# MomentsInGraphics/vulkan_renderer

Hardware: NVIDIA H100
Metric: Msamples/s (pixels x spp) at 1920x1080x64spp; achieved HBM GB/s vs roofline (higher is better)
Workload: dtype f32

## Files before the change

__graft_entry__.py:

```python
import hashlib
import os
import shutil
import subprocess
import sys

ROOT = os.path.dirname(os.path.abspath(__file__))
PKG = os.path.join(ROOT, "vulkan_renderer_b200")
CSRC = os.path.join(PKG, "csrc")
LIB = os.path.join(PKG, "libvkr_b200.so")
NVCC = shutil.which("nvcc") or "/usr/local/cuda/bin/nvcc"
HOST_CXX = "/usr/bin/g++"

NVCC_FLAGS = [
	"-gencode", "arch=compute_90a,code=sm_90a", "-lineinfo", "-O3", "-std=c++17",
	"-fmad=false", "-prec-div=true", "-prec-sqrt=true", "-ftz=false",
	"-ccbin", HOST_CXX, "-Xcompiler", "-fPIC,-O2,-ffp-contract=off,-fopenmp,-Wall,-Wno-unused-function",
	"-I", os.path.join(ROOT, "include"),
]
NVCC_FLAGS += [f for f in os.environ.get("VKR_EXTRA_NVCC", "").split() if f]
CUDA_INCLUDE =os.path.join(os.path.dirname(os.path.dirname(os.path.realpath(NVCC))), "include")
HOST_FLAGS = ["-O2", "-std=c++17", "-fPIC", "-ffp-contract=off", "-fopenmp", "-Wall", "-Wno-unused-function", "-Wno-unused-result",
	"-I", os.path.join(ROOT, "include"), "-I", os.path.join(ROOT, "shim"), "-I", CUDA_INCLUDE]
CUDA_SOURCES = ["vkr_gbuffer_kernel.cu", "vkr_api.cu", "vkr_exchange.cu", "vkr_lbvh_gpu.cu"]
SHADING_KERNEL_BOUNDS = [4, 5, 6, 7, 8]
RELATED_WORK_KERNEL_BOUNDS = [3, 4, 5, 6, 7]
HOST_SOURCES = ["vkr_host.cpp", "vkr_bvh.cpp", "vkr_lbvh.cpp", "vkr_output.cpp", "vkr_textures.cpp"]


def _run(cmd, **kw):
	proc = subprocess.run(cmd, stdout=subprocess.PIPE, stderr=subprocess.STDOUT, text=True, **kw)
	if proc.returncode != 0:
		sys.stderr.write(proc.stdout)
		raise RuntimeError("command failed: %s" % " ".join(cmd))
	return proc.stdout


def _newer(target, sources):
	if not os.path.exists(target):
		return True
	t = os.path.getmtime(target)
	return any(os.path.getmtime(s) > t for s in sources)


def _all_headers():
	out = []
	for d in (CSRC, os.path.join(ROOT, "include"), os.path.join(ROOT, "shim"), os.path.join(ROOT, "shim", "vulkan")):
		if os.path.isdir(d):
			out += [os.path.join(d, f) for f in os.listdir(d) if f.endswith((".h", ".cuh", ".inc"))]
	return out


def build_library(verbose=False):
	obj_dir = os.path.join(PKG, "build")
	os.makedirs(obj_dir, exist_ok=True)
	headers = _all_headers()
	objects = []
	sources = [(s, [], s + ".o") for s in CUDA_SOURCES + HOST_SOURCES if os.path.exists(os.path.join(CSRC, s))]
	sources += [("vkr_shading_kernel.cu", ["-DVKR_MAXP_TU=%d" % k], "vkr_shading_kernel_maxp%d.cu.o" % k) for k in SHADING_KERNEL_BOUNDS]
	sources += [("vkr_shading_kernel.cu", ["-DVKR_MAXP_TU=5", "-DVKR_TRACE_STATS=1"], "vkr_shading_kernel_stats_maxp5.cu.o")]
	sources += [("vkr_textured_light_kernel.cu", ["-DVKR_MAXP_TU=%d" % k], "vkr_textured_light_kernel_maxp%d.cu.o" % k) for k in SHADING_KERNEL_BOUNDS]
	sources += [("vkr_related_work_kernel.cu", ["-DVKR_MAXV_TU=%d" % k], "vkr_related_work_kernel_maxv%d.cu.o" % k) for k in RELATED_WORK_KERNEL_BOUNDS]
	sources += [("vkr_textured_related_work_kernel.cu", ["-DVKR_MAXV_TU=%d" % k], "vkr_textured_related_work_kernel_maxv%d.cu.o" % k) for k in RELATED_WORK_KERNEL_BOUNDS]
	procs = []
	for src, defines, obj_name in sources:
		path = os.path.join(CSRC, src)
		obj = os.path.join(obj_dir, obj_name)
		objects.append(obj)
		if _newer(obj, [path] + headers):
			if src.endswith(".cu"):
				cmd = [NVCC] + NVCC_FLAGS + defines + (["-Xptxas", "-v"] if verbose else []) + ["-c", path, "-o", obj]
			else:
				cmd = [HOST_CXX] + HOST_FLAGS + ["-c", path, "-o", obj]
			procs.append((obj_name, subprocess.Popen(cmd, stdout=subprocess.PIPE, stderr=subprocess.STDOUT, text=True)))
	failed = False
	for src, proc in procs:
		out, _ = proc.communicate()
		if proc.returncode != 0:
			sys.stderr.write("---- %s\n%s\n" % (src, out))
			failed = True
		elif verbose:
			sys.stdout.write("---- %s\n%s\n" % (src, out))
	if failed:
		raise RuntimeError("nvcc failed")
	if _newer(LIB, objects):
		_run([NVCC, "-shared", "-o", LIB] + objects + ["-ccbin", HOST_CXX, "-Xcompiler", "-fopenmp", "-lgomp", "-cudart", "static"])
	return LIB


def build_device_on_host():
	src = os.path.join(ROOT, "tests", "device_on_host.cpp")
	out = os.path.join(ROOT, "tests", "build", "libdevice_on_host.so")
	os.makedirs(os.path.dirname(out), exist_ok=True)
	if _newer(out, [src] + _all_headers()):
		_run([HOST_CXX, "-O2", "-std=c++17", "-fPIC", "-shared", "-ffp-contract=off", "-mfma", "-mavx2", "-mf16c", "-Wall", "-Wno-unused-function", "-Wno-unknown-pragmas",
			"-I", CSRC, src, "-o", out])
	return out


def build_oracle():
	_run(["make", "-C", os.path.join(ROOT, "oracle")])
	ref_recipe = os.path.join(ROOT, "oracle", "build_ref.py")
	if os.path.isdir("/root/reference/src") and os.path.exists(ref_recipe):
		_run([sys.executable, ref_recipe])


def build():
	build_library()
	build_oracle()
	build_device_on_host()
	sys.path.insert(0, ROOT)
	import vulkan_renderer_b200


def smoke():
	sys.path.insert(0, ROOT)
	from tests import harness as H
	from vulkan_renderer_b200 import api
	if not os.path.exists(LIB):
		raise RuntimeError("libvkr_b200.so has not been built; there is no CPU fallback")
	width, height = 128, 96
	info = H.dataset("cornell")
	oi = H.OracleInputs(info)
	frame = H.open_frame(info, cuda_device=0)
	try:
		frame.configure(sample_count=2, strategy=api.STRATEGY_DIFFUSE_SPECULAR_MIS, heuristic=api.MIS_OPTIMAL_CLAMPED, trace_shadow_rays=1)
		constants = frame.constants(width, height)
		vis, gb = frame.gbuffer_host(width, height)
		out = frame.shade_host(width, height, gb)
		ref, rays = oi.shade(H.oracle_config(frame, width, height), constants, gb)
	finally:
		frame.close()
	cmp = H.compare_radiance(out, ref, rel=1.0e-5)
	print("smoke: %dx%d Cornell frame, %d oracle shadow rays, %s" % (width, height, rays, cmp))
	if cmp["bad_pixels"] or cmp["nan_mismatch"] or not np_any_lit(out):
		raise RuntimeError("smoke test failed: %s" % cmp)


def np_any_lit(image):
	import numpy as np
	return bool(np.isfinite(image).all() and (image[..., :3] > 0).any())


if __name__ == "__main__":
	build_library(verbose="-v" in sys.argv)
	build_oracle()
	build_device_on_host()
	print("built", LIB)
```

vulkan_renderer_b200/csrc/vkr_ray_stream.cuh:

```cuda
#pragma once
#include "vkr_trace.cuh"
#include "vkr_anchor.cuh"

namespace vkr {

#ifndef VKR_ANCHORED
#define VKR_ANCHORED 0
#endif

#ifndef VKR_RING
#define VKR_RING 256
#endif
constexpr int kRing = VKR_RING;
constexpr unsigned kFullMask = 0xffffffffu;
#ifndef VKR_TRACE_GROUPS
#define VKR_TRACE_GROUPS 2
#endif
constexpr int kShadeWarps = 4, kTraceWarps = 4 * VKR_TRACE_GROUPS;
constexpr unsigned kPending = 0xffu;
#ifndef VKR_BVH_WIDTH
#define VKR_BVH_WIDTH 2
#endif
#ifndef VKR_NODE_LOOP_MIN_LANES
#define VKR_NODE_LOOP_MIN_LANES 16
#endif
constexpr int kNodeLoopMinLanes = VKR_NODE_LOOP_MIN_LANES;
#ifndef VKR_REFILL_MIN_LANES
#define VKR_REFILL_MIN_LANES 1
#endif
#ifndef VKR_LEAN_NODE_STEP
#define VKR_LEAN_NODE_STEP (!VKR_ANCHORED && VKR_BVH_WIDTH == 2)
#endif
#ifndef VKR_LEAF_ONCE
#define VKR_LEAF_ONCE 0
#endif
#ifndef VKR_LEAF_POSTPONE
#define VKR_LEAF_POSTPONE 1
#endif
#ifndef VKR_STACK_TOP_IN_REGISTER
#define VKR_STACK_TOP_IN_REGISTER 0
#endif
#ifndef VKR_TRACE_RELOAD_RAY
#define VKR_TRACE_RELOAD_RAY 0
#endif
#ifndef VKR_SHADING_LOCKSTEP
#define VKR_SHADING_LOCKSTEP 0
#endif
#ifndef VKR_NODE_LOOP_CHECK_EVERY
#define VKR_NODE_LOOP_CHECK_EVERY 1
#endif
VKR_DEV void shading_lockstep_barrier() {
#if defined(__CUDA_ARCH__)
	asm volatile("bar.sync 1, 128;" ::: "memory");
#endif
}
#ifndef VKR_QUANTISED_NODES
#define VKR_QUANTISED_NODES 0
#endif
#ifndef VKR_INTERLEAVED_NODES
#define VKR_INTERLEAVED_NODES (!VKR_ANCHORED && !VKR_QUANTISED_NODES && VKR_BVH_WIDTH == 2)
#endif
#if VKR_ANCHORED && VKR_BVH_WIDTH != 2
#error "anchored rays walk node pairs"
#endif
#if VKR_LEAN_NODE_STEP && (VKR_ANCHORED || VKR_BVH_WIDTH != 2 || VKR_STACK_TOP_IN_REGISTER)
#error "the predicated node step: not with anchored rays, 4-wide nodes or the stack top in a register (-DVKR_LEAN_NODE_STEP=0)"
#endif
#if VKR_INTERLEAVED_NODES && (VKR_ANCHORED || VKR_QUANTISED_NODES || VKR_BVH_WIDTH != 2)
#error "interleaved node pairs: not with anchored rays, quantised pairs or 4-wide nodes"
#endif
#ifndef VKR_RESOLVE_SLEEP_NS
#define VKR_RESOLVE_SLEEP_NS 512
#endif

#ifdef VKR_TRACE_STATS
#define VKR_STAT(x) (++(x))
#define VKR_STAT_ADD(x, n) ((x) += (n))
#else
#define VKR_STAT(x) ((void) 0)
#define VKR_STAT_ADD(x, n) ((void) 0)
#endif
VKR_DEV void stat_flush(unsigned long long* stats, int index, unsigned value) {
#if defined(VKR_TRACE_STATS) && defined(__CUDA_ARCH__)
	value = __reduce_add_sync(kFullMask, value);
	if ((threadIdx.x & 31) == 0 && value != 0u && stats) atomicAdd(stats + index, (unsigned long long) value);
#endif
}

enum : int {
	S_DX = 0, S_DY = kRing, S_DZ = 2 * kRing, S_TMAX = 3 * kRing,
	S_CX = 4 * kRing, S_CY = 5 * kRing, S_CZ = 6 * kRing,
	S_OX = 7 * kRing, S_OY = 8 * kRing, S_OZ = 9 * kRing
};
VKR_DEV constexpr int stream_bytes_at(bool optimal) { return (optimal ? 10 : 7) * kRing; }
VKR_DEV constexpr int stream_origin_at(bool optimal) { return stream_bytes_at(optimal) + 2 * kRing / 4; }
VKR_DEV constexpr int stream_control_at(bool optimal) { return stream_origin_at(optimal) + 96; }
VKR_DEV constexpr int stream_mask_at(bool optimal) { return stream_control_at(optimal) + 4; }
VKR_DEV constexpr int stream_path_at(bool optimal) { return stream_mask_at(optimal) + kRing; }
VKR_DEV constexpr int stream_cone_at(bool optimal) { return stream_path_at(optimal) + 32 * (kPathLevels + 2); }
VKR_DEV constexpr size_t stream_floats_per_warp(bool optimal) { return VKR_ANCHORED ? (size_t) stream_cone_at(optimal) + 6 * 32 : (size_t) stream_control_at(optimal) + 4; }

VKR_DEV uint32_t smem_addr(const void* p) { return (uint32_t) __cvta_generic_to_shared(p); }
VKR_DEV uint32_t lds_u32(uint32_t a) { uint32_t v; asm volatile("ld.shared.u32 %0, [%1];" : "=r"(v) : "r"(a) : "memory"); return v; }
VKR_DEV void sts_u32(uint32_t a, uint32_t v) { asm volatile("st.shared.u32 [%0], %1;" :: "r"(a), "r"(v) : "memory"); }
VKR_DEV float lds_f(uint32_t a) { float v; asm volatile("ld.shared.f32 %0, [%1];" : "=f"(v) : "r"(a) : "memory"); return v; }
VKR_DEV void sts_f(uint32_t a, float v) { asm volatile("st.shared.f32 [%0], %1;" :: "r"(a), "f"(v) : "memory"); }
VKR_DEV unsigned lds_u8(uint32_t a) { unsigned v; asm volatile("ld.shared.u8 %0, [%1];" : "=r"(v) : "r"(a) : "memory"); return v; }
VKR_DEV void sts_u8(uint32_t a, unsigned v) { asm volatile("st.shared.u8 [%0], %1;" :: "r"(a), "r"(v) : "memory"); }
VKR_DEV int ld_acquire(uint32_t a) { int v; asm volatile("ld.acquire.cta.shared::cta.b32 %0, [%1];" : "=r"(v) : "r"(a) : "memory"); return v; }
VKR_DEV void st_release(uint32_t a, int v) { asm volatile("st.release.cta.shared::cta.b32 [%0], %1;" :: "r"(a), "r"(v) : "memory"); }
VKR_DEV unsigned ld_acquire_u8(uint32_t a) { unsigned v; asm volatile("ld.acquire.cta.shared::cta.u8 %0, [%1];" : "=r"(v) : "r"(a) : "memory"); return v; }
VKR_DEV void st_release_u8(uint32_t a, unsigned v) { asm volatile("st.release.cta.shared::cta.u8 [%0], %1;" :: "r"(a), "r"(v) : "memory"); }
VKR_DEV int atom_add_shared(uint32_t a, int v) { int old; asm volatile("atom.relaxed.cta.shared::cta.add.s32 %0, [%1], %2;" : "=r"(old) : "r"(a), "r"(v) : "memory"); return old; }

struct ray_producer {
	uint32_t base;
	int fill;
	int resolved;
#ifdef VKR_TRACE_STATS
	unsigned stat_resolve_polls, stat_candidates;
#endif
	bool cone_set;
	bool lockstep;
};

struct pixel_sum {
	f3 color;
	f3 light;
	float inv_samples;
	unsigned submit_parity, resolve_parity;
	bool pushed;
};
VKR_DEV void close_light(pixel_sum& acc) {
	acc.color = acc.color + acc.light * acc.inv_samples;
	acc.light = make3(0.0f, 0.0f, 0.0f);
}

template <bool OPTIMAL>
VKR_DEV void resolve_chunk(ray_producer& q, int lane, pixel_sum& acc) {
	const uint32_t bytes = q.base + 4u * stream_bytes_at(OPTIMAL);
	const int first = q.resolved;
	const int n = min(32, q.fill - first);
	const uint32_t slot = (uint32_t) (first + lane) & (kRing - 1);
	const bool valid = lane < n;
	while (true) {
		const unsigned r = valid ? ld_acquire_u8(bytes + kRing + slot) : 0u;
		if (!__any_sync(kFullMask, r == kPending)) break;
		VKR_STAT(q.stat_resolve_polls);
		__nanosleep(VKR_RESOLVE_SLEEP_NS);
	}
	const unsigned own = valid ? (lds_u8(bytes + slot) & 31u) : 32u;
	unsigned mine = __ballot_sync(kFullMask, valid);
#pragma unroll
	for (int b = 0; b != 5; ++b) {
		const unsigned bits = __ballot_sync(kFullMask, (own >> b) & 1u);
		mine &= ((lane >> b) & 1) ? bits : ~bits;
	}
	while (mine) {
		const uint32_t e = (uint32_t) (first + __ffs(mine) - 1) & (kRing - 1);
		mine &= mine - 1;
		const uint32_t a = q.base + 4u * e;
		const unsigned parity = lds_u8(bytes + e) & 32u;
		if (parity != acc.resolve_parity) { close_light(acc); acc.resolve_parity = parity; }
		if (!lds_u8(bytes + kRing + e)) acc.light = acc.light + make3(lds_f(a + 4u * S_CX), lds_f(a + 4u * S_CY), lds_f(a + 4u * S_CZ));
		else if (OPTIMAL) acc.light = acc.light + make3(lds_f(a + 4u * S_OX), lds_f(a + 4u * S_OY), lds_f(a + 4u * S_OZ));
	}
	q.resolved = first + n;
	__syncwarp(kFullMask);
}

#define OPTIMAL_STREAM_HAS_CONE(q) ((q).cone_set)
template <bool TRACE, bool OPTIMAL>
VKR_DEV void set_light_cone(ray_producer& q, int lane, bool on, f3 origin, const unsigned char* vertices, int vertex_count, const float4* __restrict__ nodes) {
#if VKR_ANCHORED
	if constexpr (TRACE) {
		q.cone_set = false;
		if (on) {
			const light_cone c = make_light_cone(origin, vertices, vertex_count);
			if (c.enabled) {
				const uint32_t path = q.base + 4u * (uint32_t) stream_path_at(OPTIMAL) + 4u * (uint32_t) lane;
				const int count = (int) lds_u32(path + 128u * (uint32_t) (kPathLevels + 1));
				const uint32_t siblings = cull_siblings(nodes, origin, c, count, [&](int k) { return lds_u32(path + 128u * (uint32_t) k); });
				const uint32_t ca = q.base + 4u * (uint32_t) stream_cone_at(OPTIMAL) + 4u * (uint32_t) lane;
				sts_f(ca, c.axis.x); sts_f(ca + 128u, c.axis.y); sts_f(ca + 256u, c.axis.z); sts_f(ca + 384u, c.cos2_valid); sts_f(ca + 512u, c.len2_valid); sts_u32(ca + 640u, siblings);
				q.cone_set = true;
			}
		}
	}
#endif
}
template <bool TRACE, bool OPTIMAL>
VKR_DEV void submit(ray_producer& q, int lane, bool has, bool need_trace, f3 dir_world, float tmax, f3 c_visible, f3 c_occluded, pixel_sum& acc, bool finish) {
	if constexpr (!TRACE) {
		if (has) {
			if (need_trace) acc.light = acc.light + c_visible;
			else if (OPTIMAL) acc.light = acc.light + c_occluded;
		}
		if (finish) close_light(acc);
	}
	else {
		const bool push = has && (need_trace || OPTIMAL);
		if (has) VKR_STAT(q.stat_candidates);
		const unsigned mask = __ballot_sync(kFullMask, push);
		if (mask) {
			const int k = __popc(mask);
			while (q.fill + k - q.resolved > kRing) resolve_chunk<OPTIMAL>(q, lane, acc);
			if (push) {
				const uint32_t e = (uint32_t) (q.fill + __popc(mask & ((1u << lane) - 1u))) & (kRing - 1);
				const uint32_t a = q.base + 4u * e;
				sts_f(a + 4u * S_DX, dir_world.x); sts_f(a + 4u * S_DY, dir_world.y); sts_f(a + 4u * S_DZ, dir_world.z); sts_f(a + 4u * S_TMAX, tmax);
				sts_f(a + 4u * S_CX, c_visible.x); sts_f(a + 4u * S_CY, c_visible.y); sts_f(a + 4u * S_CZ, c_visible.z);
				if (OPTIMAL) { sts_f(a + 4u * S_OX, c_occluded.x); sts_f(a + 4u * S_OY, c_occluded.y); sts_f(a + 4u * S_OZ, c_occluded.z); }
				const uint32_t bytes = q.base + 4u * stream_bytes_at(OPTIMAL);
				sts_u8(bytes + e, (unsigned) lane | acc.submit_parity | (need_trace ? 0u : 128u));
				sts_u8(bytes + kRing + e, kPending);
#if VKR_ANCHORED
				{
					uint32_t siblings = kAllSiblings;
					if (OPTIMAL_STREAM_HAS_CONE(q)) {
						const uint32_t ca = q.base + 4u * (uint32_t) stream_cone_at(OPTIMAL) + 4u * (uint32_t) lane;
						const f3 axis = make3(lds_f(ca), lds_f(ca + 128u), lds_f(ca + 256u));
						const float aw = dot(axis, dir_world), ww = dot(dir_world, dir_world);
						if (aw > 0.0f && aw * aw >= lds_f(ca + 384u) * ww && tmax * tmax * ww <= lds_f(ca + 512u)) siblings = lds_u32(ca + 640u);
					}
					sts_u32(q.base + 4u * (uint32_t) stream_mask_at(OPTIMAL) + 4u * e, siblings);
				}
#endif
				acc.pushed = true;
			}
			q.fill += k;
			__syncwarp(kFullMask);
			if (lane == 0) st_release(q.base + 4u * stream_control_at(OPTIMAL) + 4u, q.fill);
		}
		if (finish && acc.pushed) { acc.submit_parity ^= 32u; acc.pushed = false; }
	}
}

template <bool OPTIMAL>
VKR_DEV void close_stream(ray_producer& q, int lane, pixel_sum& acc, unsigned long long* stats = nullptr) {
	while (q.resolved != q.fill) resolve_chunk<OPTIMAL>(q, lane, acc);
	close_light(acc);
	__syncwarp(kFullMask);
	if (lane == 0) st_release(q.base + 4u * stream_control_at(OPTIMAL) + 8u, q.fill);
#ifdef VKR_TRACE_STATS
	stat_flush(stats, 10, lane == 0 ? (unsigned) q.fill : 0u);
	stat_flush(stats, 11, lane == 0 ? q.stat_resolve_polls : 0u);
	stat_flush(stats, 12, q.stat_candidates);
#endif
}

template <bool OPTIMAL>
VKR_DEV void trace_stream(const uint32_t base, const float4* __restrict__ nodes, const float4* __restrict__ tris, const uint32_t stack_bottom, int lane, unsigned long long* stats = nullptr,
	const uint4* __restrict__ nodes_q = nullptr, f3 grid_min = f3(), f3 grid_scale = f3(), const float4* __restrict__ nodes_i = nullptr)
{
#ifdef VKR_TRACE_STATS
	unsigned st_rays = 0, st_hits = 0, st_cache_hits = 0, st_visits = 0, st_leaves = 0, st_tris = 0, st_iters = 0, st_node_iters = 0, st_known = 0, st_polls = 0, st_siblings = 0;
#endif
	const unsigned lt_mask = (1u << lane) - 1u;
	const float tmin = 1.0e-3f;
	const uint32_t bytes = base + 4u * stream_bytes_at(OPTIMAL);
	const uint32_t origin = base + 4u * stream_origin_at(OPTIMAL);
	const uint32_t control = base + 4u * stream_control_at(OPTIMAL);
	uint32_t top = stack_bottom;
#if VKR_STACK_TOP_IN_REGISTER
	int stack_top = kTraversalDone;
	auto push = [&](int v) { asm volatile("st.shared.b32 [%0], %1;" :: "r"(top), "r"(stack_top) : "memory"); top += 128u; stack_top = v; };
	auto pop = [&]() { const int v = stack_top; top -= 128u; asm volatile("ld.shared.b32 %0, [%1];" : "=r"(stack_top) : "r"(top) : "memory"); return v; };
#else
	auto push = [&](int v) { asm volatile("st.shared.b32 [%0], %1;" :: "r"(top), "r"(v) : "memory"); top += 128u; };
	auto pop = [&]() { int v; top -= 128u; asm volatile("ld.shared.b32 %0, [%1];" : "=r"(v) : "r"(top) : "memory"); return v; };
#endif
	int ticket = -1;
	uint32_t entry = 0;
	bool active = false;
	bool hit = false;
	bool finished = false;
	int node = kTraversalDone, leaf = 0;
#if VKR_ANCHORED
	uint32_t pending = 0u;
	uint32_t path = 0u;
#endif
	int cached_triangle = -1;
#if VKR_TRACE_RELOAD_RAY
	unsigned own_lane = 0;
#else
	f3 o = make3(0.0f, 0.0f, 0.0f), d = make3(0.0f, 0.0f, 1.0f);
#endif
	float tmax = 0.0f;
#if VKR_QUANTISED_NODES
	ray_grid r = make_ray_grid(make3(0.0f, 0.0f, 0.0f), make3(0.0f, 0.0f, 1.0f), grid_min, grid_scale);
#else
	ray_slabs r = make_slabs<false>(make3(0.0f, 0.0f, 0.0f), make3(0.0f, 0.0f, 1.0f));
#endif
	while (true) {
		const bool wants = !active && ticket < 0 && !finished;
		const unsigned want = __ballot_sync(kFullMask, wants);
#if VKR_REFILL_MIN_LANES > 1
		const unsigned busy = __ballot_sync(kFullMask, active);
		const bool refill = busy == 0u || __popc(~busy) >= VKR_REFILL_MIN_LANES;
#else
		const bool refill = true;
#endif
		if (want && refill) {
			const int leader = __ffs(want) - 1;
			int first = 0;
			if (lane == leader) first = atom_add_shared(control, __popc(want));
			first = __shfl_sync(kFullMask, first, leader);
			if (wants) ticket = first + __popc(want & lt_mask);
		}
		if (ticket >= 0 && refill) {
			if (ticket < ld_acquire(control + 4u)) {
				entry = (uint32_t) ticket & (kRing - 1);
				ticket = -1;
				const unsigned own = lds_u8(bytes + entry);
				if (own & 128u) {
					VKR_STAT(st_known);
					st_release_u8(bytes + kRing + entry, 1u);
				}
				else {
					VKR_STAT(st_rays);
					const uint32_t oa = origin + 4u * (own & 31u), ea = base + 4u * entry;
#if VKR_TRACE_RELOAD_RAY
					own_lane = own & 31u;
					const f3 o = make3(lds_f(oa), lds_f(oa + 128u), lds_f(oa + 256u));
					const f3 d = make3(lds_f(ea + 4u * S_DX), lds_f(ea + 4u * S_DY), lds_f(ea + 4u * S_DZ));
#else
					o = make3(lds_f(oa), lds_f(oa + 128u), lds_f(oa + 256u));
					d = make3(lds_f(ea + 4u * S_DX), lds_f(ea + 4u * S_DY), lds_f(ea + 4u * S_DZ));
#endif
					tmax = lds_f(ea + 4u * S_TMAX);
					active = true;
					hit = false;
					node = kTraversalDone; leaf = 0;
#if VKR_ANCHORED
					pending = 0u;
#endif
					float t;
#ifdef VKR_NULL_TRACE
					if (false) {
#else
					if (tmax > tmin) {
#endif
#ifndef VKR_NO_OCCLUDER_CACHE
						if (cached_triangle >= 0 && ray_triangle(tris + 3 * (size_t) cached_triangle, o, d, tmin, tmax, &t)) { hit = true; VKR_STAT(st_cache_hits); }
#else
						if (false) {}
#endif
						else {
#if VKR_QUANTISED_NODES
							r = make_ray_grid(o, d, grid_min, grid_scale);
#else
							r = make_slabs<false>(o, d);
#endif
							top = stack_bottom; push(kTraversalDone);
#if VKR_ANCHORED
							path = base + 4u * (uint32_t) stream_path_at(OPTIMAL) + 4u * (own & 31u);
							const uint32_t count = lds_u32(path + 128u * (uint32_t) (kPathLevels + 1));
							pending = lds_u32(base + 4u * (uint32_t) stream_mask_at(OPTIMAL) + 4u * entry) & ((1u << count) - 1u);
							node = (int) lds_u32(path + 128u * (uint32_t) kPathLevels);
							if (node < 0) { leaf = node; node = pop(); }
#else
							node = 0;
#endif
						}
					}
				}
			}
			else {
				const int end = ld_acquire(control + 8u);
				if (end >= 0 && ticket >= end) { finished = true; ticket = -1; }
			}
		}
		if (!__any_sync(kFullMask, active)) {
			if (__all_sync(kFullMask, finished)) break;
			if (lane == 0) VKR_STAT(st_polls);
			__nanosleep(100);
			continue;
		}
		if (lane == 0) VKR_STAT(st_iters);
#if VKR_NODE_LOOP_CHECK_EVERY > 1
		unsigned node_steps = 0u;
#endif
#if VKR_BVH_WIDTH == 4
		while (node >= 0 && node != kTraversalDone) {
			VKR_STAT(st_visits);
			if ((__activemask() & lt_mask) == 0u) VKR_STAT(st_node_iters);
			node = bvh4_descend_step(nodes, node, r, tmin, tmax, push);
			if (node == kTraversalDone) node = pop();
			if (node < 0 && leaf == 0) {
				leaf = node;
				node = pop();
			}
			if (kNodeLoopMinLanes > 0 && __popc(__activemask()) < kNodeLoopMinLanes) break;
		}
#else
#if VKR_ANCHORED
		while (node >= 0 && (node != kTraversalDone || (pending != 0u && active && !hit))) {
			int skip = 2;
			if (node == kTraversalDone) {
				const int k = 31 - __clz((int) pending);
				pending &= ~(1u << k);
				const uint32_t e = lds_u32(path + 128u * (uint32_t) k);
				node = (int) (e >> 1); skip = (int) (e & 1u);
				top = stack_bottom; push(kTraversalDone);
				VKR_STAT(st_siblings);
			}
#else
		while (node >= 0 && node != kTraversalDone) {
			const int skip = 2;
#endif
			float tn0, tn1;
			VKR_STAT(st_visits);
			if ((__activemask() & lt_mask) == 0u) VKR_STAT(st_node_iters);
#if VKR_QUANTISED_NODES
			float4 q0, q1;
			ldg_32_bytes(reinterpret_cast<const float4*>(nodes_q) + 2 * (size_t) node, q0, q1);
			const int ref0 = __float_as_int(q1.z), ref1 = __float_as_int(q1.w);
			const bool h0 = ray_box_grid(__float_as_uint(q0.x), __float_as_uint(q0.y), __float_as_uint(q0.z), r, tmin, tmax, &tn0);
			const bool h1 = ray_box_grid(__float_as_uint(q0.w), __float_as_uint(q1.x), __float_as_uint(q1.y), r, tmin, tmax, &tn1);
#elif VKR_INTERLEAVED_NODES
			const float4* nd = reinterpret_cast<const float4*>(reinterpret_cast<const char*>(nodes_i) + (size_t) ((uint32_t) node << 6));
			float4 q0, q1, q2, q3;
			ldg_32_bytes(nd, q0, q1); ldg_32_bytes(nd + 2, q2, q3);
			const int ref0 = __float_as_int(q3.x), ref1 = __float_as_int(q3.y);
			bool h0, h1;
			{
				const float a[8] = { q0.x, q0.y, q0.z, q0.w, q1.x, q1.y, q1.z, q1.w }, b[4] = { q2.x, q2.y, q2.z, q2.w };
				ray_box_pair(a, b, r, tmin, tmax, &h0, &h1, &tn0, &tn1);
			}
#else
#if VKR_LEAN_NODE_STEP
			const float4* nd = reinterpret_cast<const float4*>(reinterpret_cast<const char*>(nodes) + (size_t) ((uint32_t) node << 6));
#else
			const float4* nd = nodes + 4 * (size_t) node;
#endif
			float4 q0, q1, q2, q3;
			ldg_32_bytes(nd, q0, q1); ldg_32_bytes(nd + 2, q2, q3);
			const int ref0 = __float_as_int(q3.x), ref1 = __float_as_int(q3.y);
			const bool h0 = ray_box(q0.x, q0.y, q0.z, q0.w, q1.x, q1.y, r, tmin, tmax, &tn0) && skip != 0;
			const bool h1 = ray_box(q1.z, q1.w, q2.x, q2.y, q2.z, q2.w, r, tmin, tmax, &tn1) && skip != 1;
#endif
#if VKR_LEAN_NODE_STEP
			{
				const int h0i = h0, h1i = h1;
				asm volatile("{\n\t.reg .pred h0, h1, both, none, second, take;\n\t.reg .b32 far;\n\t"
					"setp.ne.b32 h0, %3, 0;\n\tsetp.ne.b32 h1, %4, 0;\n\t"
					"setp.lt.f32 second, %6, %5;\n\t"
					"and.pred both, h0, h1;\n\t"
					"or.pred none, h0, h1;\n\tnot.pred none, none;\n\t"
					"not.pred take, h0;\n\tor.pred second, second, take;\n\tand.pred second, second, h1;\n\t"
					"selp.b32 %1, %8, %7, second;\n\tselp.b32 far, %7, %8, second;\n\t"
					"@both st.shared.b32 [%0], far;\n\t@both add.u32 %0, %0, 128;\n\t"
					"@none sub.u32 %0, %0, 128;\n\t@none ld.shared.b32 %1, [%0];\n\t"
#if VKR_LEAF_POSTPONE
					"setp.lt.s32 take, %1, 0;\n\tsetp.eq.and.s32 take, %2, 0, take;\n\t"
					"@take mov.b32 %2, %1;\n\t@take sub.u32 %0, %0, 128;\n\t@take ld.shared.b32 %1, [%0];\n\t"
#endif
					"}"
					: "+r"(top), "=&r"(node), "+r"(leaf) : "r"(h0i), "r"(h1i), "f"(tn0), "f"(tn1), "r"(ref0), "r"(ref1) : "memory");
			}
#else
			if (h0 && h1) {
				const bool swap = tn1 < tn0;
				node = swap ? ref1 : ref0;
				push(swap ? ref0 : ref1);
			}
			else if (h0) node = ref0;
			else if (h1) node = ref1;
			else node = pop();
#endif
#if !VKR_LEAN_NODE_STEP && VKR_LEAF_POSTPONE
			if (node < 0 && leaf == 0) {
				leaf = node;
				node = pop();
			}
#endif
#if VKR_NODE_LOOP_CHECK_EVERY > 1
			if ((++node_steps & (VKR_NODE_LOOP_CHECK_EVERY - 1)) != 0) continue;
#endif
			if (kNodeLoopMinLanes > 0 && __popc(__activemask()) < kNodeLoopMinLanes) break;
		}
#endif
		__syncwarp(kFullMask);
#if !VKR_LEAF_POSTPONE
		if (active && node < 0 && leaf == 0) { leaf = node; node = pop(); }
#endif
#if VKR_LEAF_ONCE
		if (leaf != 0) {
#else
		while (leaf != 0) {
#endif
			const int first = (leaf & 0x7fffffff) >> 4, count = leaf & 15;
			float t;
#if VKR_TRACE_RELOAD_RAY
			const uint32_t oa = origin + 4u * own_lane, ea = base + 4u * entry;
			const f3 o = make3(lds_f(oa), lds_f(oa + 128u), lds_f(oa + 256u));
			const f3 d = make3(lds_f(ea + 4u * S_DX), lds_f(ea + 4u * S_DY), lds_f(ea + 4u * S_DZ));
#endif
			VKR_STAT(st_leaves); VKR_STAT_ADD(st_tris, (unsigned) count);
			for (int i = 0; i != count; ++i)
				if (ray_triangle(tris + 3 * (size_t) (first + i), o, d, tmin, tmax, &t)) { hit = true; cached_triangle = first + i; }
			leaf = 0;
			if (hit) node = kTraversalDone;
			else if (node < 0) {
				leaf = node;
				node = pop();
			}
		}
#if VKR_ANCHORED
		if (active && node == kTraversalDone && leaf == 0 && (hit || pending == 0u)) {
#else
		if (active && node == kTraversalDone && leaf == 0) {
#endif
			st_release_u8(bytes + kRing + entry, hit ? 1u : 0u);
			if (hit) VKR_STAT(st_hits);
			active = false;
		}
		__syncwarp(kFullMask);
	}
#ifdef VKR_TRACE_STATS
	stat_flush(stats, 0, st_rays); stat_flush(stats, 1, st_hits); stat_flush(stats, 2, st_cache_hits); stat_flush(stats, 3, st_visits); stat_flush(stats, 4, st_leaves);
	stat_flush(stats, 5, st_tris); stat_flush(stats, 6, st_iters); stat_flush(stats, 7, st_node_iters); stat_flush(stats, 8, st_known); stat_flush(stats, 9, st_polls); stat_flush(stats, 13, st_siblings);
#endif
}

}
```

vulkan_renderer_b200/csrc/vkr_trace.cuh:

```cuda
#pragma once
#include "vkr_device_math.cuh"

namespace vkr {

struct bvh_view {
	const float4* nodes;
	const float4* tris;
	const uint32_t* tri_ids;
	uint32_t tri_count;
};

constexpr int kMaxStackDepth = 64;
constexpr int kTraversalDone = 0x7fffffff;

VKR_DEV bool ray_triangle(const float4* __restrict__ tri, f3 o, f3 d, float tmin, float tmax, float* out_t) {
	const float4 a = __ldg(tri), b = __ldg(tri + 1), c = __ldg(tri + 2);
	const f3 p0 = make3(a.x, a.y, a.z);
	const f3 e1 = make3(a.w, b.x, b.y);
	const f3 e2 = make3(b.z, b.w, c.x);
	const f3 pv = cross(d, e2);
	const float det = dot(e1, pv);
	if (det == 0.0f) return false;
	const float inv_det = 1.0f / det;
	const f3 tv = o - p0;
	const float u = dot(tv, pv) * inv_det;
	if (!(u >= 0.0f && u <= 1.0f)) return false;
	const f3 qv = cross(tv, e1);
	const float v = dot(d, qv) * inv_det;
	if (!(v >= 0.0f && u + v <= 1.0f)) return false;
	const float t = dot(e2, qv) * inv_det;
	if (!(t > tmin && t < tmax)) return false;
	*out_t = t;
	return true;
}

VKR_DEV void ldg_32_bytes(const float4* __restrict__ p, float4& a, float4& b) {
	a = __ldg(p); b = __ldg(p + 1);
}

VKR_DEV float unguarded_slab_reciprocal(float x) {
#if defined(__CUDA_ARCH__) && !defined(VKR_EXACT_SLAB_RECIPROCAL)
	float y; asm("rcp.approx.ftz.f32 %0, %1;" : "=f"(y) : "f"(x)); return y;
#else
	return 1.0f / x;
#endif
}
VKR_DEV float slab_reciprocal(float x) {
	const float y = unguarded_slab_reciprocal(x);
	return (fabsf(x) < 5.421010862427522e-20f) ? copysignf(__int_as_float(0x7f800000), x) : y;
}

struct ray_slabs { f3 id, oid; };
template <bool GUARDED = true>
VKR_DEV ray_slabs make_slabs(f3 o, f3 d) {
	ray_slabs r;
	if (GUARDED) r.id = make3(slab_reciprocal(d.x), slab_reciprocal(d.y), slab_reciprocal(d.z));
	else r.id = make3(unguarded_slab_reciprocal(d.x), unguarded_slab_reciprocal(d.y), unguarded_slab_reciprocal(d.z));
	r.oid = make3(o.x * r.id.x, o.y * r.id.y, o.z * r.id.z);
	return r;
}

VKR_DEV bool ray_box(float cx, float cy, float cz, float hx, float hy, float hz, const ray_slabs& r, float tmin, float tmax, float* t_near) {
	const float mx = fmaf(cx, r.id.x, -r.oid.x), my = fmaf(cy, r.id.y, -r.oid.y), mz = fmaf(cz, r.id.z, -r.oid.z);
	const float ax = fabsf(r.id.x), ay = fabsf(r.id.y), az = fabsf(r.id.z);
	const float tn = fmaxf(fmaxf(fmaf(-hx, ax, mx), fmaf(-hy, ay, my)), fmaxf(fmaf(-hz, az, mz), tmin));
	const float tf = fminf(fminf(fmaf(hx, ax, mx), fmaf(hy, ay, my)), fminf(fmaf(hz, az, mz), tmax));
	*t_near = tn;
	return tn <= tf;
}

VKR_DEV void interleave_node_pair(const float4* __restrict__ pair, float* out16) {
	const float4 q0 = pair[0], q1 = pair[1], q2 = pair[2], q3 = pair[3];
	out16[0] = q0.x; out16[1] = q1.z; out16[2] = q0.y; out16[3] = q1.w; out16[4] = q0.z; out16[5] = q2.x;
	out16[6] = q0.w; out16[7] = q2.y; out16[8] = q1.x; out16[9] = q2.z; out16[10] = q1.y; out16[11] = q2.w;
	out16[12] = q3.x; out16[13] = q3.y; out16[14] = 0.0f; out16[15] = 0.0f;
}
VKR_DEV void fma_pair(float& d0, float& d1, float a0, float a1, float s, float c0, float c1) {
	d0 = fmaf(a0, s, c0); d1 = fmaf(a1, s, c1);
}
VKR_DEV void ray_box_pair(const float (&a)[8], const float (&b)[4], const ray_slabs& r, float tmin, float tmax, bool* h0, bool* h1, float* tn0, float* tn1) {
	float mx0, mx1, my0, my1, mz0, mz1, nx0, nx1, ny0, ny1, nz0, nz1, fx0, fx1, fy0, fy1, fz0, fz1;
	const float nox = -r.oid.x, noy = -r.oid.y, noz = -r.oid.z;
	fma_pair(mx0, mx1, a[0], a[1], r.id.x, nox, nox); fma_pair(my0, my1, a[2], a[3], r.id.y, noy, noy); fma_pair(mz0, mz1, a[4], a[5], r.id.z, noz, noz);
	const float ax = fabsf(r.id.x), ay = fabsf(r.id.y), az = fabsf(r.id.z);
	fma_pair(nx0, nx1, a[6], a[7], -ax, mx0, mx1); fma_pair(ny0, ny1, b[0], b[1], -ay, my0, my1); fma_pair(nz0, nz1, b[2], b[3], -az, mz0, mz1);
	fma_pair(fx0, fx1, a[6], a[7], ax, mx0, mx1); fma_pair(fy0, fy1, b[0], b[1], ay, my0, my1); fma_pair(fz0, fz1, b[2], b[3], az, mz0, mz1);
	*tn0 = fmaxf(fmaxf(nx0, ny0), fmaxf(nz0, tmin)); *tn1 = fmaxf(fmaxf(nx1, ny1), fmaxf(nz1, tmin));
	const float tf0 = fminf(fminf(fx0, fy0), fminf(fz0, tmax)), tf1 = fminf(fminf(fx1, fy1), fminf(fz1, tmax));
	*h0 = *tn0 <= tf0; *h1 = *tn1 <= tf1;
}
VKR_DEV bool occluded_interleaved(const float* __restrict__ pairs16, const float4* __restrict__ tris, f3 o, f3 d, float tmin, float tmax, int* stack, int stride, int* visits) {
	if (!(tmax > tmin)) return false;
	const ray_slabs r = make_slabs(o, d);
	int sp = 0, node = 0;
	float t, tn0, tn1;
	while (true) {
		if (node < 0) {
			const int first = (node & 0x7fffffff) >> 4, count = node & 15;
			for (int i = 0; i != count; ++i)
				if (ray_triangle(tris + 3 * (size_t) (first + i), o, d, tmin, tmax, &t)) return true;
			if (sp == 0) return false;
			--sp; node = stack[sp * stride];
			continue;
		}
		if (visits) ++*visits;
		const float* w = pairs16 + 16 * (size_t) node;
		const float a[8] = { w[0], w[1], w[2], w[3], w[4], w[5], w[6], w[7] }, b[4] = { w[8], w[9], w[10], w[11] };
		bool h0, h1;
		ray_box_pair(a, b, r, tmin, tmax, &h0, &h1, &tn0, &tn1);
		const int ref0 = __float_as_int(w[12]), ref1 = __float_as_int(w[13]);
		if (h0 && h1) { const bool swap = tn1 < tn0; stack[sp * stride] = swap ? ref0 : ref1; ++sp; node = swap ? ref1 : ref0; }
		else if (h0) node = ref0;
		else if (h1) node = ref1;
		else { if (sp == 0) return false; --sp; node = stack[sp * stride]; }
	}
}

struct ray_grid { f3 id, c; unsigned near_x, near_y, near_z; };
constexpr unsigned kGridMagic = 0x4B000000u;
VKR_DEV ray_grid make_ray_grid(f3 o, f3 d, f3 grid_min, f3 grid_scale) {
	ray_grid g;
	const f3 og = make3((o.x - grid_min.x) * grid_scale.x, (o.y - grid_min.y) * grid_scale.y, (o.z - grid_min.z) * grid_scale.z);
	const f3 dg = make3(d.x * grid_scale.x, d.y * grid_scale.y, d.z * grid_scale.z);
	g.id = make3(slab_reciprocal(dg.x), slab_reciprocal(dg.y), slab_reciprocal(dg.z));
	g.c = make3(-fmaf(8388608.0f, g.id.x, og.x * g.id.x), -fmaf(8388608.0f, g.id.y, og.y * g.id.y), -fmaf(8388608.0f, g.id.z, og.z * g.id.z));
	g.near_x = (dg.x < 0.0f) ? 0x7632u : 0x7610u; g.near_y = (dg.y < 0.0f) ? 0x7632u : 0x7610u; g.near_z = (dg.z < 0.0f) ? 0x7632u : 0x7610u;
	return g;
}
VKR_DEV float grid_plane(unsigned word, unsigned selector) {
#if defined(__CUDA_ARCH__)
	return __uint_as_float(__byte_perm(word, kGridMagic, selector));
#else
	return __uint_as_float(kGridMagic | ((selector == 0x7632u) ? (word >> 16) : (word & 0xffffu)));
#endif
}
VKR_DEV bool ray_box_grid(unsigned wx, unsigned wy, unsigned wz, const ray_grid& g, float tmin, float tmax, float* t_near) {
	const float nx = fmaf(grid_plane(wx, g.near_x), g.id.x, g.c.x), ny = fmaf(grid_plane(wy, g.near_y), g.id.y, g.c.y), nz = fmaf(grid_plane(wz, g.near_z), g.id.z, g.c.z);
	const float fx = fmaf(grid_plane(wx, g.near_x ^ 0x0022u), g.id.x, g.c.x), fy = fmaf(grid_plane(wy, g.near_y ^ 0x0022u), g.id.y, g.c.y), fz = fmaf(grid_plane(wz, g.near_z ^ 0x0022u), g.id.z, g.c.z);
	const float tn = fmaxf(fmaxf(nx, ny), fmaxf(nz, tmin));
	const float tf = fminf(fminf(fx, fy), fminf(fz, tmax));
	*t_near = tn;
	return tn <= tf;
}
VKR_DEV void quantise_node_pair(const float4* __restrict__ pair, const float* grid_min, const float* grid_scale, unsigned* out8) {
	const float4 q0 = pair[0], q1 = pair[1], q2 = pair[2], q3 = pair[3];
	const float c[2][3] = { { q0.x, q0.y, q0.z }, { q1.z, q1.w, q2.x } }, h[2][3] = { { q0.w, q1.x, q1.y }, { q2.y, q2.z, q2.w } };
	for (int k = 0; k != 2; ++k)
		for (int a = 0; a != 3; ++a) {
			float lo = floorf(((c[k][a] - h[k][a]) - grid_min[a]) * grid_scale[a]) - 1.0f, hi = ceilf(((c[k][a] + h[k][a]) - grid_min[a]) * grid_scale[a]) + 1.0f;
			if (h[k][a] < 0.0f) { lo = 65535.0f; hi = 0.0f; }
			lo = fminf(fmaxf(lo, 0.0f), 65535.0f); hi = fminf(fmaxf(hi, 0.0f), 65535.0f);
			out8[3 * k + a] = (unsigned) lo | ((unsigned) hi << 16);
		}
	out8[6] = __float_as_uint(q3.x); out8[7] = __float_as_uint(q3.y);
}
VKR_DEV bool occluded_grid(const unsigned* __restrict__ pairs8, const float4* __restrict__ tris, const float* grid_min, const float* grid_scale, f3 o, f3 d, float tmin, float tmax, int* stack, int stride, int* visits) {
	if (!(tmax > tmin)) return false;
	const ray_grid g = make_ray_grid(o, d, make3(grid_min[0], grid_min[1], grid_min[2]), make3(grid_scale[0], grid_scale[1], grid_scale[2]));
	int sp = 0, node = 0;
	float t, tn0, tn1;
	while (true) {
		if (node < 0) {
			const int first = (node & 0x7fffffff) >> 4, count = node & 15;
			for (int i = 0; i != count; ++i)
				if (ray_triangle(tris + 3 * (size_t) (first + i), o, d, tmin, tmax, &t)) return true;
			if (sp == 0) return false;
			--sp; node = stack[sp * stride];
			continue;
		}
		if (visits) ++*visits;
		const unsigned* w = pairs8 + 8 * (size_t) node;
		const bool h0 = ray_box_grid(w[0], w[1], w[2], g, tmin, tmax, &tn0), h1 = ray_box_grid(w[3], w[4], w[5], g, tmin, tmax, &tn1);
		const int ref0 = (int) w[6], ref1 = (int) w[7];
		if (h0 && h1) { const bool swap = tn1 < tn0; stack[sp * stride] = swap ? ref0 : ref1; ++sp; node = swap ? ref1 : ref0; }
		else if (h0) node = ref0;
		else if (h1) node = ref1;
		else { if (sp == 0) return false; --sp; node = stack[sp * stride]; }
	}
}

VKR_DEV bool occluded(const bvh_view& bvh, f3 o, f3 d, float tmin, float tmax, int* stack, int stride) {
	if (!(tmax > tmin)) return false;
	const ray_slabs r = make_slabs(o, d);
	int sp = 0;
	int node = 0;
	float t, tn0, tn1;
	while (true) {
		const float4* n = bvh.nodes + 4 * (size_t) node;
		const float4 q0 = __ldg(n), q1 = __ldg(n + 1), q2 = __ldg(n + 2), q3 = __ldg(n + 3);
		const int ref0 = __float_as_int(q3.x), ref1 = __float_as_int(q3.y);
		bool h0 = ray_box(q0.x, q0.y, q0.z, q0.w, q1.x, q1.y, r, tmin, tmax, &tn0);
		bool h1 = ray_box(q1.z, q1.w, q2.x, q2.y, q2.z, q2.w, r, tmin, tmax, &tn1);
		if (h0 && ref0 < 0) {
			const int first = (ref0 & 0x7fffffff) >> 4, count = ref0 & 15;
			for (int i = 0; i != count; ++i)
				if (ray_triangle(bvh.tris + 3 * (size_t) (first + i), o, d, tmin, tmax, &t)) return true;
			h0 = false;
		}
		if (h1 && ref1 < 0) {
			const int first = (ref1 & 0x7fffffff) >> 4, count = ref1 & 15;
			for (int i = 0; i != count; ++i)
				if (ray_triangle(bvh.tris + 3 * (size_t) (first + i), o, d, tmin, tmax, &t)) return true;
			h1 = false;
		}
		if (h0 && h1) { stack[sp * stride] = ref1; ++sp; node = ref0; }
		else if (h0) node = ref0;
		else if (h1) node = ref1;
		else {
			if (sp == 0) return false;
			--sp; node = stack[sp * stride];
		}
	}
}

template <class Push>
VKR_DEV int bvh4_descend_step(const float4* __restrict__ nodes4, int node, const ray_slabs& r, float tmin, float tmax, Push&& push) {
	const float4* nd = nodes4 + 8 * (size_t) node;
	float4 q0, q1, q2, q3, q4, q5, q6, q7;
	ldg_32_bytes(nd, q0, q1); ldg_32_bytes(nd + 2, q2, q3); ldg_32_bytes(nd + 4, q4, q5); ldg_32_bytes(nd + 6, q6, q7);
	const int ref0 = __float_as_int(q6.x), ref1 = __float_as_int(q6.y), ref2 = __float_as_int(q6.z), ref3 = __float_as_int(q6.w);
	float tn0, tn1, tn2, tn3;
	const bool h0 = ray_box(q0.x, q0.y, q0.z, q0.w, q1.x, q1.y, r, tmin, tmax, &tn0);
	const bool h1 = ray_box(q1.z, q1.w, q2.x, q2.y, q2.z, q2.w, r, tmin, tmax, &tn1);
	const bool h2 = ray_box(q3.x, q3.y, q3.z, q3.w, q4.x, q4.y, r, tmin, tmax, &tn2);
	const bool h3 = ray_box(q4.z, q4.w, q5.x, q5.y, q5.z, q5.w, r, tmin, tmax, &tn3);
	int best = -1; float best_t = 0.0f;
	if (h0) { best = 0; best_t = tn0; }
	if (h1 && (best < 0 || tn1 < best_t)) { best = 1; best_t = tn1; }
	if (h2 && (best < 0 || tn2 < best_t)) { best = 2; best_t = tn2; }
	if (h3 && (best < 0 || tn3 < best_t)) { best = 3; best_t = tn3; }
	if (h0 && best != 0) push(ref0);
	if (h1 && best != 1) push(ref1);
	if (h2 && best != 2) push(ref2);
	if (h3 && best != 3) push(ref3);
	return (best < 0) ? kTraversalDone : ((best == 0) ? ref0 : ((best == 1) ? ref1 : ((best == 2) ? ref2 : ref3)));
}

VKR_DEV bool occluded4(const float4* __restrict__ nodes4, const float4* __restrict__ tris, f3 o, f3 d, float tmin, float tmax, int* stack, int stride, int* steps) {
	if (!(tmax > tmin)) return false;
	const ray_slabs r = make_slabs(o, d);
	int sp = 0;
	int node = 0;
	float t;
	auto push = [&](int ref) { stack[sp * stride] = ref; ++sp; };
	while (true) {
		if (node < 0) {
			const int first = (node & 0x7fffffff) >> 4, count = node & 15;
			for (int i = 0; i != count; ++i)
				if (ray_triangle(tris + 3 * (size_t) (first + i), o, d, tmin, tmax, &t)) return true;
			node = kTraversalDone;
		}
		else {
			if (steps) ++*steps;
			node = bvh4_descend_step(nodes4, node, r, tmin, tmax, push);
		}
		if (node == kTraversalDone) {
			if (sp == 0) return false;
			--sp; node = stack[sp * stride];
		}
	}
}

VKR_DEV int closest_hit(const bvh_view& bvh, f3 o, f3 d, float tmin, float tmax, int* stack, int stride) {
	const ray_slabs r = make_slabs(o, d);
	int sp = 0;
	int node = 0;
	int best = -1;
	float best_t = tmax;
	float t, tn0, tn1;
	while (true) {
		const float4* n = bvh.nodes + 4 * (size_t) node;
		const float4 q0 = __ldg(n), q1 = __ldg(n + 1), q2 = __ldg(n + 2), q3 = __ldg(n + 3);
		const int ref0 = __float_as_int(q3.x), ref1 = __float_as_int(q3.y);
		bool h0 = ray_box(q0.x, q0.y, q0.z, q0.w, q1.x, q1.y, r, tmin, best_t, &tn0);
		bool h1 = ray_box(q1.z, q1.w, q2.x, q2.y, q2.z, q2.w, r, tmin, best_t, &tn1);
#pragma unroll
		for (int c = 0; c != 2; ++c) {
			const int ref = c ? ref1 : ref0;
			const bool h = c ? h1 : h0;
			if (h && ref < 0) {
				const int first = (ref & 0x7fffffff) >> 4, count = ref & 15;
				for (int i = 0; i != count; ++i) {
					if (ray_triangle(bvh.tris + 3 * (size_t) (first + i), o, d, tmin, __int_as_float(0x7f800000), &t)) {
						const int id_ = (int) __ldg(bvh.tri_ids + first + i);
						if (t < best_t || (t == best_t && best >= 0 && id_ < best)) { best_t = t; best = id_; }
					}
				}
				if (c) h1 = false; else h0 = false;
			}
		}
		if (h0 && h1) {
			const bool swap = tn1 < tn0;
			stack[sp * stride] = swap ? ref0 : ref1; ++sp; node = swap ? ref1 : ref0;
		}
		else if (h0) node = ref0;
		else if (h1) node = ref1;
		else {
			if (sp == 0) return best;
			--sp; node = stack[sp * stride];
		}
	}
}

}
```

Baseline: 335.2.

## Use DPX integer min/max for slab tests with clamped reciprocals

Replaces the float min/max reductions in the paired ray-box slab test with signed-integer three-way min/max (Hopper DPX __vimax3_s32/__vimin3_s32) on the float bit patterns. Reciprocals are clamped to a finite range so the bit patterns stay well ordered. The interleaved traversal path now uses the clamped slabs. The change also lowers the node-loop minimum lane threshold and simplifies the traversal loop condition to one unsigned compare. Integer ordering of float bits is only correct for non-negative values or consistent signs, so correctness depends on tmin being non-negative and on how negative slab distances compare, and it may not match float semantics in edge cases.

```diff
diff --git a/__graft_entry__.py b/__graft_entry__.py
--- a/__graft_entry__.py
+++ b/__graft_entry__.py
@@ -88,12 +88,13 @@
 
 
 def build_device_on_host():
-	src = os.path.join(ROOT, "tests", "device_on_host.cpp")
-	out = os.path.join(ROOT, "tests", "build", "libdevice_on_host.so")
-	os.makedirs(os.path.dirname(out), exist_ok=True)
-	if _newer(out, [src] + _all_headers()):
-		_run([HOST_CXX, "-O2", "-std=c++17", "-fPIC", "-shared", "-ffp-contract=off", "-mfma", "-mavx2", "-mf16c", "-Wall", "-Wno-unused-function", "-Wno-unknown-pragmas",
-			"-I", CSRC, src, "-o", out])
+	for name in ("dpx_slab_on_host", "device_on_host"):
+		src = os.path.join(ROOT, "tests", name + ".cpp")
+		out = os.path.join(ROOT, "tests", "build", "lib%s.so" % name)
+		os.makedirs(os.path.dirname(out), exist_ok=True)
+		if _newer(out, [src] + _all_headers()):
+			_run([HOST_CXX, "-O2", "-std=c++17", "-fPIC", "-shared", "-ffp-contract=off", "-mfma", "-mavx2", "-mf16c", "-Wall", "-Wno-unused-function", "-Wno-unknown-pragmas",
+				"-I", CSRC, src, "-o", out])
 	return out
 
 
diff --git a/vulkan_renderer_b200/csrc/vkr_ray_stream.cuh b/vulkan_renderer_b200/csrc/vkr_ray_stream.cuh
--- a/vulkan_renderer_b200/csrc/vkr_ray_stream.cuh
+++ b/vulkan_renderer_b200/csrc/vkr_ray_stream.cuh
@@ -22,7 +22,7 @@
 #define VKR_BVH_WIDTH 2
 #endif
 #ifndef VKR_NODE_LOOP_MIN_LANES
-#define VKR_NODE_LOOP_MIN_LANES 16
+#define VKR_NODE_LOOP_MIN_LANES 8
 #endif
 constexpr int kNodeLoopMinLanes = VKR_NODE_LOOP_MIN_LANES;
 #ifndef VKR_REFILL_MIN_LANES
@@ -349,6 +349,8 @@
 						else {
 #if VKR_QUANTISED_NODES
 							r = make_ray_grid(o, d, grid_min, grid_scale);
+#elif VKR_INTERLEAVED_NODES
+							r = make_clamped_slabs(o, d);
 #else
 							r = make_slabs<false>(o, d);
 #endif
@@ -406,7 +408,7 @@
 				VKR_STAT(st_siblings);
 			}
 #else
-		while (node >= 0 && node != kTraversalDone) {
+		while ((unsigned) node < (unsigned) kTraversalDone) {
 			const int skip = 2;
 #endif
 			float tn0, tn1;
@@ -426,7 +428,7 @@
 			bool h0, h1;
 			{
 				const float a[8] = { q0.x, q0.y, q0.z, q0.w, q1.x, q1.y, q1.z, q1.w }, b[4] = { q2.x, q2.y, q2.z, q2.w };
-				ray_box_pair(a, b, r, tmin, tmax, &h0, &h1, &tn0, &tn1);
+				ray_box_pair<true>(a, b, r, tmin, tmax, &h0, &h1, &tn0, &tn1);
 			}
 #else
 #if VKR_LEAN_NODE_STEP
diff --git a/vulkan_renderer_b200/csrc/vkr_trace.cuh b/vulkan_renderer_b200/csrc/vkr_trace.cuh
--- a/vulkan_renderer_b200/csrc/vkr_trace.cuh
+++ b/vulkan_renderer_b200/csrc/vkr_trace.cuh
@@ -59,6 +59,33 @@
 	r.oid = make3(o.x * r.id.x, o.y * r.id.y, o.z * r.id.z);
 	return r;
 }
+VKR_DEV float clamped_slab_reciprocal(float x) {
+	const float big = 18446744073709551616.0f;
+	return fminf(fmaxf(unguarded_slab_reciprocal(x), -big), big);
+}
+VKR_DEV ray_slabs make_clamped_slabs(f3 o, f3 d) {
+	ray_slabs r;
+	r.id = make3(clamped_slab_reciprocal(d.x), clamped_slab_reciprocal(d.y), clamped_slab_reciprocal(d.z));
+	r.oid = make3(o.x * r.id.x, o.y * r.id.y, o.z * r.id.z);
+	return r;
+}
+
+VKR_DEV int imax3_s32(int a, int b, int c) {
+#if defined(__CUDA_ARCH__)
+	return __vimax3_s32(a, b, c);
+#else
+	const int m = (a > b) ? a : b; return (m > c) ? m : c;
+#endif
+}
+VKR_DEV int imin3_s32(int a, int b, int c) {
+#if defined(__CUDA_ARCH__)
+	return __vimin3_s32(a, b, c);
+#else
+	const int m = (a < b) ? a : b; return (m < c) ? m : c;
+#endif
+}
+VKR_DEV int imax_s32(int a, int b) { return (a > b) ? a : b; }
+VKR_DEV int imin_s32(int a, int b) { return (a < b) ? a : b; }
 
 VKR_DEV bool ray_box(float cx, float cy, float cz, float hx, float hy, float hz, const ray_slabs& r, float tmin, float tmax, float* t_near) {
 	const float mx = fmaf(cx, r.id.x, -r.oid.x), my = fmaf(cy, r.id.y, -r.oid.y), mz = fmaf(cz, r.id.z, -r.oid.z);
@@ -78,6 +105,7 @@
 VKR_DEV void fma_pair(float& d0, float& d1, float a0, float a1, float s, float c0, float c1) {
 	d0 = fmaf(a0, s, c0); d1 = fmaf(a1, s, c1);
 }
+template <bool DPX = false>
 VKR_DEV void ray_box_pair(const float (&a)[8], const float (&b)[4], const ray_slabs& r, float tmin, float tmax, bool* h0, bool* h1, float* tn0, float* tn1) {
 	float mx0, mx1, my0, my1, mz0, mz1, nx0, nx1, ny0, ny1, nz0, nz1, fx0, fx1, fy0, fy1, fz0, fz1;
 	const float nox = -r.oid.x, noy = -r.oid.y, noz = -r.oid.z;
@@ -85,13 +113,24 @@
 	const float ax = fabsf(r.id.x), ay = fabsf(r.id.y), az = fabsf(r.id.z);
 	fma_pair(nx0, nx1, a[6], a[7], -ax, mx0, mx1); fma_pair(ny0, ny1, b[0], b[1], -ay, my0, my1); fma_pair(nz0, nz1, b[2], b[3], -az, mz0, mz1);
 	fma_pair(fx0, fx1, a[6], a[7], ax, mx0, mx1); fma_pair(fy0, fy1, b[0], b[1], ay, my0, my1); fma_pair(fz0, fz1, b[2], b[3], az, mz0, mz1);
-	*tn0 = fmaxf(fmaxf(nx0, ny0), fmaxf(nz0, tmin)); *tn1 = fmaxf(fmaxf(nx1, ny1), fmaxf(nz1, tmin));
-	const float tf0 = fminf(fminf(fx0, fy0), fminf(fz0, tmax)), tf1 = fminf(fminf(fx1, fy1), fminf(fz1, tmax));
+	float tf0, tf1;
+	if (DPX) {
+		const int lo = __float_as_int(tmin), hi = __float_as_int(tmax);
+		*tn0 = __int_as_float(imax_s32(imax3_s32(__float_as_int(nx0), __float_as_int(ny0), __float_as_int(nz0)), lo));
+		*tn1 = __int_as_float(imax_s32(imax3_s32(__float_as_int(nx1), __float_as_int(ny1), __float_as_int(nz1)), lo));
+		tf0 = __int_as_float(imin_s32(imin3_s32(__float_as_int(fx0), __float_as_int(fy0), __float_as_int(fz0)), hi));
+		tf1 = __int_as_float(imin_s32(imin3_s32(__float_as_int(fx1), __float_as_int(fy1), __float_as_int(fz1)), hi));
+	}
+	else {
+		*tn0 = fmaxf(fmaxf(nx0, ny0), fmaxf(nz0, tmin)); *tn1 = fmaxf(fmaxf(nx1, ny1), fmaxf(nz1, tmin));
+		tf0 = fminf(fminf(fx0, fy0), fminf(fz0, tmax)); tf1 = fminf(fminf(fx1, fy1), fminf(fz1, tmax));
+	}
 	*h0 = *tn0 <= tf0; *h1 = *tn1 <= tf1;
 }
+template <bool DPX = false>
 VKR_DEV bool occluded_interleaved(const float* __restrict__ pairs16, const float4* __restrict__ tris, f3 o, f3 d, float tmin, float tmax, int* stack, int stride, int* visits) {
 	if (!(tmax > tmin)) return false;
-	const ray_slabs r = make_slabs(o, d);
+	const ray_slabs r = DPX ? make_clamped_slabs(o, d) : make_slabs(o, d);
 	int sp = 0, node = 0;
 	float t, tn0, tn1;
 	while (true) {
@@ -107,7 +146,7 @@
 		const float* w = pairs16 + 16 * (size_t) node;
 		const float a[8] = { w[0], w[1], w[2], w[3], w[4], w[5], w[6], w[7] }, b[4] = { w[8], w[9], w[10], w[11] };
 		bool h0, h1;
-		ray_box_pair(a, b, r, tmin, tmax, &h0, &h1, &tn0, &tn1);
+		ray_box_pair<DPX>(a, b, r, tmin, tmax, &h0, &h1, &tn0, &tn1);
 		const int ref0 = __float_as_int(w[12]), ref1 = __float_as_int(w[13]);
 		if (h0 && h1) { const bool swap = tn1 < tn0; stack[sp * stride] = swap ? ref0 : ref1; ++sp; node = swap ? ref1 : ref0; }
 		else if (h0) node = ref0;
```

Result: faster. 348.4, median of 6 (+3.9%).
